# PRBonn/RAP

Measured on AMD Instinct MI355X. Metric: registered points/sec @20 flow steps, 2-view N=4096, higher is better.
Workload: dtype f32; 1 GPU; configs[1]: batch=32 samples/GPU x 2 views x 4096 pts, 20 Euler flow steps, rap_12 (d=512, H=8), fp32 (exact-fp32 MFMA), rigidity_forcing=on, final per-view SE(3) fit; preset=1, pairs_per_gpu=32, views=2, points_per_view=4096, flow_steps=20, num_layers=12, rigidity_forcing=True

## Files before the change

rap_amd/csrc/api.hip:

```cpp
#include "../../include/rapflow.h"
#include "half.h"
#include "kernels.h"

#include <mutex>
#include <new>
#include <vector>

static thread_local int g_last_hip_error = 0;
void rap_set_last_hip_error(int e) { g_last_hip_error = e; }

#define RAP_PROF_CLASSES 8
struct ProfRec { hipEvent_t a, b; int cls; };
static std::atomic<bool> g_prof_on{false};
static std::mutex g_prof_mu;
static std::vector<ProfRec> g_prof_recs;
static std::vector<hipEvent_t> g_prof_pool;
static size_t g_prof_pool_used = 0;
static const size_t RAP_PROF_MAX_EVENTS = 1u << 19;

static hipEvent_t prof_event() {
  if (g_prof_pool_used < g_prof_pool.size()) return g_prof_pool[g_prof_pool_used++];
  if (g_prof_pool.size() >= RAP_PROF_MAX_EVENTS) return nullptr;
  hipEvent_t e = nullptr;
  if (hipEventCreate(&e) != hipSuccess) return nullptr;
  g_prof_pool.push_back(e);
  g_prof_pool_used++;
  return e;
}
struct ProfScope {
  hipStream_t s; hipEvent_t a = nullptr, b = nullptr; int cls;
  ProfScope(hipStream_t s_, int cls_) : s(s_), cls(cls_) {
    if (!g_prof_on.load(std::memory_order_relaxed)) return;
    std::lock_guard<std::mutex> lock(g_prof_mu);
    a = prof_event(); b = prof_event();
    if (a && b) (void)hipEventRecord(a, s); else a = b = nullptr;
  }
  ~ProfScope() {
    if (a && b) {
      std::lock_guard<std::mutex> lock(g_prof_mu);
      (void)hipEventRecord(b, s); g_prof_recs.push_back({a, b, cls});
    }
  }
};
extern "C" int rap_profile_enable(int on) { g_prof_on.store(on != 0); return RAP_OK; }
extern "C" int rap_profile_reset(void) { std::lock_guard<std::mutex> lock(g_prof_mu); g_prof_recs.clear(); g_prof_pool_used = 0; return RAP_OK; }
extern "C" int rap_profile_collect_ex(float* h_ms_out, int64_t* h_count_out, int32_t n_classes) {
  if (!h_ms_out || !h_count_out || n_classes <= 0) return RAP_ERR_INVALID;
  std::lock_guard<std::mutex> lock(g_prof_mu);
  for (int c = 0; c < n_classes; ++c) { h_ms_out[c] = 0.f; h_count_out[c] = 0; }
  for (const ProfRec& r : g_prof_recs) {
    if (r.cls >= n_classes) continue;
    if (hipEventSynchronize(r.b) != hipSuccess) return RAP_ERR_HIP;
    float ms = 0.f;
    if (hipEventElapsedTime(&ms, r.a, r.b) != hipSuccess) return RAP_ERR_HIP;
    h_ms_out[r.cls] += ms; h_count_out[r.cls] += 1;
  }
  return RAP_OK;
}
extern "C" int rap_profile_collect(float* h_ms_out, int64_t* h_count_out) { return rap_profile_collect_ex(h_ms_out, h_count_out, 3); }

struct LayerW {
  const float* Wqkv[2];
  const float* Wout[2];
  const float* bout[2];
  const float* gq[2];
  const float* gk[2];
  const float* ffn_g;
  const float* ffn_b;
  const float* Wff1p;
  const float* bff1p;
  const float* Wff2;
  const float* bff2;
};

struct LayerWH {
  const u16* Wqkv[2];
  const u16* Wout[2];
  const u16* Wff1p;
  const u16* Wff2;
  float s_qkv[2] = {1.f, 1.f}, s_out[2] = {1.f, 1.f}, s_ff1 = 1.f, s_ff2 = 1.f;
  float g_v[2] = {1.f, 1.f}, g_ff1 = 1.f;
};
struct HalfWeights {
  u16* blob = nullptr;
  std::vector<LayerWH> layers;
};
#define RAP_MAX_LOGIT_BOUND 40.0f

struct rap_model {
  rap_model_desc desc;
  int d, L, H, F, E;
  int Din = 0;
  int Ks = 128;
  int dtype = RAP_DT_F32;
  bool qk_norm = true;
  int resid_dtype = RAP_DT_F32;
  HalfWeights half[4];
  float* logit_bound = nullptr;
  std::vector<uint8_t> bounded;
  int n_bounded = 0;
  float* raw = nullptr;
  float* derived = nullptr;
  const float* anchor_emb;
  const float* emb_bias;
  const float* Wstatic;
  const float* Wx;
  const float *adaW1, *adab1, *adaW2, *adab2, *adaW3, *adab3;
  std::vector<LayerW> layers;
  const float *hW0, *hb0, *hW2, *hb2, *hW4;
  mutable std::mutex cfg_mu;
};

static bool desc_ok(const rap_model_desc* d) {
  if (!d) return false;
  if (d->embed_dim <= 0 || d->embed_dim % 256 != 0 || d->embed_dim > 1024) return false;
  if (d->num_heads * 64 != d->embed_dim) return false;
  if (d->num_layers <= 0 || d->num_layers > 64) return false;
  if (d->local_feat_dim < 0 || d->local_feat_dim % 4 != 0 || d->local_feat_dim > 40) return false;
  return true;
}

extern rap_tuning_t g_rap_gemm_variant;
extern rap_tuning_t g_rap_gemm_stagger;
extern rap_tuning_t g_rap_gemm_splitk;
extern rap_tuning_t g_rap_geglu_fast;
extern rap_tuning_t g_rap_attn_split;
extern rap_tuning_t g_rap_gemm_h16_variant;
extern rap_tuning_t g_rap_attn_h16_variant;
extern rap_tuning_t g_rap_gemm_h16_persistent;
extern rap_tuning_t g_rap_attn_h16_dma;
extern rap_tuning_t g_rap_gemm_f32_persistent;
extern rap_tuning_t g_rap_attn_x2_wpe;
extern rap_tuning_t g_rap_attn_h16_small;
rap_tuning_t g_rap_attn_lpt = 1;
rap_tuning_t g_rap_x2_min_rows = 1024;
rap_tuning_t g_rap_small_fused = 1;
extern rap_tuning_t g_rap_ring_blocks;
rap_tuning_t g_rap_fuse_qknorm = 1;
struct TuningRow { int32_t key; rap_tuning_t* var; int n_values; int32_t values[7]; };
static const TuningRow kTuning[] = {
#ifdef RAP_ABLATION_BUILD
  {0, &g_rap_gemm_variant, 3, {16, 32, 48}},
  {2, &g_rap_gemm_h16_variant, 3, {0, 1, 14}},
  {3, &g_rap_attn_h16_variant, 2, {0, 5}},
  {4, &g_rap_gemm_stagger, 3, {0, 1, 2}},
#endif
  {5, &g_rap_attn_split, 2, {0, 1}},
  {6, &g_rap_gemm_splitk, 2, {0, 1}},
  {7, &g_rap_fuse_qknorm, 2, {0, 1}},
  {9, &g_rap_geglu_fast, 2, {0, 1}},
  {11, &g_rap_gemm_h16_persistent, 2, {0, 1}},
  {12, &g_rap_gemm_f32_persistent, 2, {0, 1}},
  {13, &g_rap_attn_h16_dma, 2, {0, 1}},
  {15, &g_rap_attn_lpt, 2, {0, 1}},
  {16, &g_rap_attn_x2_wpe, 2, {2, 4}},
  {17, &g_rap_x2_min_rows, -1, {}},
  {18, &g_rap_ring_blocks, -1, {}},
  {19, &g_rap_small_fused, 2, {0, 1}},
  {20, &g_rap_attn_h16_small, 7, {0, 1, 2, 64, 128, 66, 130}},
};
extern "C" int rap_set_tuning(int32_t key, int32_t value) {
  for (const TuningRow& r : kTuning) {
    if (r.key != key) continue;
    bool ok = r.n_values < 0 && value >= 0;
    for (int i = 0; i < r.n_values; ++i) ok = ok || r.values[i] == value;
    if (ok) *r.var = value;
    return ok ? RAP_OK : RAP_ERR_INVALID;
  }
  return RAP_ERR_INVALID;
}

extern "C" int rap_version(void) { return RAPFLOW_ABI_VERSION; }
extern "C" int rap_last_hip_error(void) { return g_last_hip_error; }

static bool in_dim_ok(int32_t in_dim) { return in_dim >= 0 && in_dim <= 512 && in_dim % 4 == 0; }
extern "C" int64_t rap_weight_count(const rap_model_desc* desc) { return rap_weight_count_latent(desc, 0); }
extern "C" int64_t rap_weight_count_latent(const rap_model_desc* desc, int32_t in_dim) {
  if (!desc_ok(desc) || !in_dim_ok(in_dim)) return -1;
  const int64_t d = desc->embed_dim, L = desc->num_layers, H = desc->num_heads, E = 147 + desc->local_feat_dim + in_dim;
  int64_t n = 2 * d + d * E + d;
  const int64_t attn = (d * 256 + d) + (d * d + d) + (2 * d * d + 2 * d) + 3 * d * d + (d * d + d) + 2 * H * 64;
  const int64_t layer = 2 * attn + 2 * d + (8 * d * d + 8 * d) + (4 * d * d + d);
  n += L * layer;
  n += (d * d + d) + (d / 2 * d + d / 2) + 3 * (d / 2);
  return n;
}

static int ensure_logit_bounds(rap_model* m, hipStream_t stream);

extern "C" int rap_model_create(const rap_model_desc* desc, const float* d_weights, int64_t n_floats, void* stream_,
                                rap_model** out) {
  return rap_model_create_latent(desc, 0, d_weights, n_floats, stream_, out);
}
extern "C" int rap_model_create_latent(const rap_model_desc* desc, int32_t in_dim, const float* d_weights, int64_t n_floats, void* stream_,
                                       rap_model** out) {
  if (!out) return RAP_ERR_INVALID;
  *out = nullptr;
  if (!desc_ok(desc) || !in_dim_ok(in_dim) || !d_weights) return RAP_ERR_INVALID;
  if (n_floats != rap_weight_count_latent(desc, in_dim)) return RAP_ERR_INVALID;
  hipStream_t stream = (hipStream_t)stream_;
  rap_model* m = new (std::nothrow) rap_model();
  if (!m) return RAP_ERR_ALLOC;
  m->desc = *desc;
  const int d = m->d = desc->embed_dim, L = m->L = desc->num_layers, H = m->H = desc->num_heads;
  m->F = desc->local_feat_dim;
  m->Din = in_dim;
  const int Ks = m->Ks = 128 + (in_dim + 31) / 32 * 32;
  const int E = m->E = 147 + m->F + m->Din;
  if (hipMalloc((void**)&m->raw, (size_t)n_floats * sizeof(float)) != hipSuccess) { delete m; return RAP_ERR_ALLOC; }
  const size_t n_ada = (size_t)2 * L * ((size_t)d * 256 + d + (size_t)d * d + d + (size_t)2 * d * d + 2 * d);
  const size_t n_ff1 = (size_t)L * ((size_t)8 * d * d + 8 * d);
  const size_t n_derived = (size_t)d * Ks + (size_t)d * 64 + n_ada + n_ff1;
  if (hipMalloc((void**)&m->derived, n_derived * sizeof(float)) != hipSuccess) {
    (void)hipFree(m->raw); delete m; return RAP_ERR_ALLOC;
  }
  int rc = RAP_OK;
  auto fail = [&](int code) { rap_model_destroy(m); return code; };
  if (hipMemcpyAsync(m->raw, d_weights, (size_t)n_floats * sizeof(float), hipMemcpyDeviceToDevice, stream) != hipSuccess)
    return fail(RAP_ERR_HIP);

  const float* p = m->raw;
  auto take = [&](size_t n) { const float* r = p; p += n; return r; };
  m->anchor_emb = take((size_t)2 * d);
  const float* embW = take((size_t)d * E);
  m->emb_bias = take(d);

  float* q = m->derived;
  auto carve = [&](size_t n) { float* r = q; q += n; return r; };
  float* Wstatic = carve((size_t)d * Ks);
  float* Wx = carve((size_t)d * 64);
  float* aW1 = carve((size_t)2 * L * d * 256); float* ab1 = carve((size_t)2 * L * d);
  float* aW2 = carve((size_t)2 * L * d * d);   float* ab2 = carve((size_t)2 * L * d);
  float* aW3 = carve((size_t)2 * L * 2 * d * d); float* ab3 = carve((size_t)2 * L * 2 * d);
  m->Wstatic = Wstatic; m->Wx = Wx;
  m->adaW1 = aW1; m->adab1 = ab1; m->adaW2 = aW2; m->adab2 = ab2; m->adaW3 = aW3; m->adab3 = ab3;

  if ((rc = launch_fill_zero(stream, Wstatic, (size_t)d * Ks))) return fail(rc);
  if ((rc = launch_fill_zero(stream, Wx, (size_t)d * 64))) return fail(rc);
  if ((rc = launch_copy_cols(stream, embW, E, 0, Wstatic, Ks, 0, d, 63))) return fail(rc);
  if ((rc = launch_copy_cols(stream, embW, E, 126, Wstatic, Ks, 63, d, 21))) return fail(rc);
  if ((rc = launch_copy_cols(stream, embW, E, 147, Wstatic, Ks, 84, d, m->F))) return fail(rc);
  if ((rc = launch_copy_cols(stream, embW, E, 147 + m->F, Wstatic, Ks, 128, d, m->Din))) return fail(rc);
  if ((rc = launch_copy_cols(stream, embW, E, 63, Wx, 64, 0, d, 63))) return fail(rc);

  m->layers.resize(L);
  for (int i = 0; i < L; ++i) {
    LayerW& lw = m->layers[i];
    for (int a = 0; a < 2; ++a) {
      const int j = 2 * i + a;
      const float* W1 = take((size_t)d * 256); const float* b1 = take(d);
      const float* W2 = take((size_t)d * d);   const float* b2 = take(d);
      const float* W3 = take((size_t)2 * d * d); const float* b3 = take((size_t)2 * d);
      if ((rc = launch_copy_cols(stream, W1, 256, 0, aW1 + (size_t)j * d * 256, 256, 0, d, 256))) return fail(rc);
      if ((rc = launch_copy_cols(stream, b1, d, 0, ab1 + (size_t)j * d, d, 0, 1, d))) return fail(rc);
      if ((rc = launch_copy_cols(stream, W2, d, 0, aW2 + (size_t)j * d * d, d, 0, d, d))) return fail(rc);
      if ((rc = launch_copy_cols(stream, b2, d, 0, ab2 + (size_t)j * d, d, 0, 1, d))) return fail(rc);
      if ((rc = launch_copy_cols(stream, W3, d, 0, aW3 + (size_t)j * 2 * d * d, d, 0, 2 * d, d))) return fail(rc);
      if ((rc = launch_copy_cols(stream, b3, 2 * d, 0, ab3 + (size_t)j * 2 * d, 2 * d, 0, 1, 2 * d))) return fail(rc);
      lw.Wqkv[a] = take((size_t)3 * d * d);
      lw.Wout[a] = take((size_t)d * d);
      lw.bout[a] = take(d);
      lw.gq[a] = take((size_t)H * 64);
      lw.gk[a] = take((size_t)H * 64);
    }
    lw.ffn_g = take(d);
    lw.ffn_b = take(d);
    const float* Wff1 = take((size_t)8 * d * d);
    const float* bff1 = take((size_t)8 * d);
    float* Wp = carve((size_t)8 * d * d);
    float* bp = carve((size_t)8 * d);
    if ((rc = launch_geglu_interleave(stream, Wff1, bff1, Wp, bp, 4 * d, d))) return fail(rc);
    lw.Wff1p = Wp; lw.bff1p = bp;
    lw.Wff2 = take((size_t)d * 4 * d);
    lw.bff2 = take(d);
  }
  m->hW0 = take((size_t)d * d); m->hb0 = take(d);
  m->hW2 = take((size_t)(d / 2) * d); m->hb2 = take(d / 2);
  m->hW4 = take((size_t)3 * (d / 2));
  if ((int64_t)(p - m->raw) != n_floats || (size_t)(q - m->derived) != n_derived) return fail(RAP_ERR_INVALID);
  if ((rc = ensure_logit_bounds(m, stream))) return fail(rc);
  *out = m;
  return RAP_OK;
}

extern "C" void rap_model_destroy(rap_model* m) {
  if (!m) return;
  if (m->raw) (void)hipFree(m->raw);
  if (m->derived) (void)hipFree(m->derived);
  for (int i = 0; i < 4; ++i)
    if (m->half[i].blob) (void)hipFree(m->half[i].blob);
  if (m->logit_bound) (void)hipFree(m->logit_bound);
  delete m;
}

static int ensure_logit_bounds(rap_model* m, hipStream_t stream) {
  if (m->logit_bound) return RAP_OK;
  const int n = m->L * 2 * m->H;
  if (hipMalloc((void**)&m->logit_bound, (size_t)n * sizeof(float)) != hipSuccess) { m->logit_bound = nullptr; return RAP_ERR_ALLOC; }
  for (int i = 0; i < m->L; ++i)
    for (int a = 0; a < 2; ++a) {
      const int rc = launch_qk_logit_bound(stream, m->layers[i].gq[a], m->layers[i].gk[a], m->H, m->logit_bound + (size_t)(2 * i + a) * m->H);
      if (rc) return rc;
    }
  std::vector<float> hb(n);
  RAP_HIP_CHECK(hipMemcpyAsync(hb.data(), m->logit_bound, (size_t)n * sizeof(float), hipMemcpyDeviceToHost, stream));
  RAP_HIP_CHECK(hipStreamSynchronize(stream));
  m->bounded.assign((size_t)2 * m->L, 1);
  for (int j = 0; j < 2 * m->L; ++j)
    for (int h = 0; h < m->H; ++h)
      if (!(hb[(size_t)j * m->H + h] <= RAP_MAX_LOGIT_BOUND)) m->bounded[j] = 0;
  m->n_bounded = 0;
  for (uint8_t b : m->bounded) m->n_bounded += b;
  return RAP_OK;
}

static int build_x2_weights(rap_model* m, hipStream_t stream) {
  HalfWeights& hw = m->half[RAP_DT_F32X2];
  const size_t d = m->d, L = m->L;
  const size_t per_layer = 2 * (2 * (3 * d * d + d * d) + 8 * d * d + 4 * d * d);
  const int nt = (int)(6 * L);
  float* d_max = nullptr;
  if (hipMalloc((void**)&d_max, (size_t)nt * sizeof(float)) != hipSuccess) return RAP_ERR_ALLOC;
  if (hipMalloc((void**)&hw.blob, per_layer * L * sizeof(u16)) != hipSuccess) { hw.blob = nullptr; (void)hipFree(d_max); return RAP_ERR_ALLOC; }
  int rc = RAP_OK;
  auto fail = [&](int code) { (void)hipFree(hw.blob); hw.blob = nullptr; hw.layers.clear(); (void)hipFree(d_max); return code; };
  if (hipMemsetAsync(d_max, 0, (size_t)nt * sizeof(float), stream) != hipSuccess) return fail(RAP_ERR_HIP);
  struct Item { const float* src; size_t rows, cols; };
  std::vector<Item> items;
  for (size_t i = 0; i < L; ++i) {
    const LayerW& lw = m->layers[i];
    for (int a = 0; a < 2; ++a) { items.push_back({lw.Wqkv[a], 3 * d, d}); items.push_back({lw.Wout[a], d, d}); }
    items.push_back({lw.Wff1p, 8 * d, d});
    items.push_back({lw.Wff2, d, 4 * d});
  }
  for (int k = 0; k < nt && rc == RAP_OK; ++k) rc = launch_max_abs(stream, items[k].src, items[k].rows * items[k].cols, d_max + k);
  if (rc) return fail(rc);
  std::vector<float> hmax(nt);
  if (hipMemcpyAsync(hmax.data(), d_max, (size_t)nt * sizeof(float), hipMemcpyDeviceToHost, stream) != hipSuccess) return fail(RAP_ERR_HIP);
  if (hipStreamSynchronize(stream) != hipSuccess) return fail(RAP_ERR_HIP);
  u16* q = hw.blob;
  std::vector<const u16*> planes(nt);
  std::vector<float> inv(nt);
  std::vector<int> expo(nt);
  for (int k = 0; k < nt && rc == RAP_OK; ++k) {
    if (!(hmax[k] < 3.0e38f)) return fail(RAP_ERR_INVALID);
    int e = 0;
    if (hmax[k] > 0.f) { int ex; (void)frexpf(hmax[k], &ex); e = 12 - ex; }
    e = e > 60 ? 60 : e < -60 ? -60 : e;
    expo[k] = hmax[k] > 0.f ? e : 16;
    inv[k] = ldexpf(1.0f, -e);
    planes[k] = q;
    rc = launch_x2_pack(stream, items[k].src, (long)items[k].cols, (long)items[k].rows, (int)items[k].cols, ldexpf(1.0f, e), q);
    q += 2 * items[k].rows * items[k].cols;
  }
  if (rc) return fail(rc);
  hw.layers.resize(L);
  for (size_t i = 0; i < L; ++i) {
    LayerWH& lh = hw.layers[i];
    const int k0 = (int)(6 * i);
    for (int a = 0; a < 2; ++a) {
      lh.Wqkv[a] = planes[k0 + 2 * a]; lh.s_qkv[a] = inv[k0 + 2 * a];
      { int g = expo[k0 + 2 * a] - 16; g = g > 12 ? 12 : g < -12 ? -12 : g; lh.g_v[a] = ldexpf(1.0f, g); }
      lh.Wout[a] = planes[k0 + 2 * a + 1]; lh.s_out[a] = inv[k0 + 2 * a + 1];
    }
    lh.Wff1p = planes[k0 + 4]; lh.s_ff1 = inv[k0 + 4];
    { int g = 2 * (expo[k0 + 4] - 16); g = g > 24 ? 24 : g < -24 ? -24 : g; lh.g_ff1 = ldexpf(1.0f, g); }
    lh.Wff2 = planes[k0 + 5]; lh.s_ff2 = inv[k0 + 5];
  }
  (void)hipFree(d_max);
  return RAP_OK;
}

extern "C" int rap_model_set_compute_dtype(rap_model* m, int32_t dtype, void* stream_) {
  if (!m) return RAP_ERR_INVALID;
  std::lock_guard<std::mutex> lock(m->cfg_mu);
  if (dtype == RAP_DT_F32) { m->dtype = dtype; return RAP_OK; }
  if (dtype != RAP_DT_BF16 && dtype != RAP_DT_F16 && dtype != RAP_DT_F32X2) return RAP_ERR_INVALID;
  HalfWeights& hw = m->half[dtype];
  if (!hw.blob && dtype == RAP_DT_F32X2) {
    const int rcx = build_x2_weights(m, (hipStream_t)stream_);
    if (rcx) return rcx;
  }
  if (!hw.blob) {
    hipStream_t stream = (hipStream_t)stream_;
    const size_t d = m->d, L = m->L;
    const size_t per_layer = 2 * (3 * d * d + d * d) + 8 * d * d + 4 * d * d;
    if (hipMalloc((void**)&hw.blob, per_layer * L * sizeof(u16)) != hipSuccess) { hw.blob = nullptr; return RAP_ERR_ALLOC; }
    u16* q = hw.blob;
    int rc = RAP_OK;
    auto conv = [&](const float* src, size_t n) -> const u16* {
      u16* dst = q; q += n;
      if (rc == RAP_OK) rc = launch_convert_h16(stream, dtype, src, dst, n);
      return dst;
    };
    hw.layers.resize(L);
    for (size_t i = 0; i < L; ++i) {
      const LayerW& lw = m->layers[i];
      LayerWH& lh = hw.layers[i];
      for (int a = 0; a < 2; ++a) {
        lh.Wqkv[a] = conv(lw.Wqkv[a], 3 * d * d);
        lh.Wout[a] = conv(lw.Wout[a], d * d);
      }
      lh.Wff1p = conv(lw.Wff1p, 8 * d * d);
      lh.Wff2 = conv(lw.Wff2, 4 * d * d);
    }
    if (rc != RAP_OK) { (void)hipFree(hw.blob); hw.blob = nullptr; hw.layers.clear(); return rc; }
  }
  { const int rcb = ensure_logit_bounds(m, (hipStream_t)stream_); if (rcb) return rcb; }
  m->dtype = dtype;
  return RAP_OK;
}
extern "C" int rap_model_compute_dtype(const rap_model* m) { return m ? m->dtype : RAP_ERR_INVALID; }
extern "C" int rap_model_set_residual_dtype(rap_model* m, int32_t dtype) {
  if (!m || (dtype != RAP_DT_F32 && dtype != RAP_DT_F16)) return RAP_ERR_INVALID;
  std::lock_guard<std::mutex> lock(m->cfg_mu);
  m->resid_dtype = dtype;
  return RAP_OK;
}
extern "C" int rap_model_residual_dtype(const rap_model* m) { return m ? m->resid_dtype : RAP_ERR_INVALID; }
extern "C" int rap_model_bounded_attention_launches(const rap_model* m) { return m ? (m->qk_norm ? m->n_bounded : 0) : RAP_ERR_INVALID; }
extern "C" int rap_model_set_qk_norm(rap_model* m, int32_t on) {
  if (!m) return RAP_ERR_INVALID;
  std::lock_guard<std::mutex> lock(m->cfg_mu);
  m->qk_norm = on != 0;
  return RAP_OK;
}
extern "C" int rap_model_qk_norm(const rap_model* m) { return m ? (m->qk_norm ? 1 : 0) : RAP_ERR_INVALID; }

static int eff_dtype(const rap_model* m, size_t rows) {
  return (m->dtype == RAP_DT_F32X2 && (long)rows < (long)g_rap_x2_min_rows) ? RAP_DT_F32 : m->dtype;
}

struct Workspace {
  float *base, *h, *xn, *qkv, *att, *ffmid, *ax, *v, *mod, *ada_scratch, *xt, *Rc, *tc, *tgrid;
  u16* h16;
  float *hid1, *hid2, *astatic;
  u16 *xnh, *qkh, *vth, *atth, *ffmidh;
  float* splitk_h;
  int splitk_planes;
  int vt_nblk;
  int rows;
  int dtype;
  bool qk_norm;
  double* proc_partials;
  int32_t *token_sample, *part_offsets, *attn_sort;
  int32_t *cu_batch_s, *cu_part_s;
  const int32_t* cu_part_live;
  int nseg_part, nseg_batch;
  AttnWorkItem *items_batch, *items_part;
  int max_items_batch, max_items_part;
  int attn_bq;
  int attn_kg;
  size_t total;
};

static Workspace carve_workspace(const rap_model* m, int64_t TP, int B, int nseg_part, int rows, char* basep, int force_dtype = -1) {
  Workspace w;
  const size_t d = m->d, L = m->L;
  Carver c(basep);
  const size_t T = align_up((size_t)TP, 256);
  w.rows = (int)T;
  const int dtype = w.dtype = force_dtype >= 0 ? force_dtype : eff_dtype(m, T);
// ... 450 lines not shown
```

rap_amd/csrc/attn_f32.hip:

```cpp
#include "kernels.h"

#define AQ_WAVE 64
#define AKV 64
#define KLD 68
#define VLD 64
#define ATTN_FENCE __builtin_amdgcn_sched_barrier(0x406);

__device__ __forceinline__ float xhalf_max(float v) {
  const auto r = __builtin_amdgcn_permlane32_swap(__float_as_uint(v), __float_as_uint(v), false, false);
  return fmaxf(__uint_as_float(r[0]), __uint_as_float(r[1]));
}
__device__ __forceinline__ float xhalf_sum(float v) {
  const auto r = __builtin_amdgcn_permlane32_swap(__float_as_uint(v), __float_as_uint(v), false, false);
  return __uint_as_float(r[0]) + __uint_as_float(r[1]);
}

#define ATTN_DEFER_THR 11.5f
__device__ __forceinline__ float amax3(float a, float b, float c) {
  float r;
  asm("v_max3_f32 %0, %1, %2, %3" : "=v"(r) : "v"(a), "v"(b), "v"(c));
  return r;
}

template <int NW, bool BOUNDED, bool SPLIT = false>
__global__ __launch_bounds__(64 * NW, 2) void attention_f32_kernel(const float* __restrict__ qkv, float* __restrict__ out,
                                                                  int TP, int heads, const AttnWorkItem* __restrict__ items,
                                                                  const float* __restrict__ bound, float* __restrict__ part_o,
                                                                  float* __restrict__ part_l) {
  __shared__ __attribute__((aligned(16))) float smem[2 * AKV * KLD + 2 * AKV * VLD];
  float* Ks = smem;
  float* Vs = smem + 2 * AKV * KLD;

  const int head = blockIdx.x % heads;
  const AttnWorkItem it = items[blockIdx.x / heads];
  const int len = it.seg_len;
  if (len <= 0) return;
  const int tid = threadIdx.x;
  const int lane = tid & 63, wave = tid >> 6;
  const int hi = lane >> 5, l31 = lane & 31;

  const size_t plane = (size_t)heads * TP * 64;
  const float* Qg = qkv + ((size_t)head * TP + it.seg_start) * 64;
  const float* Kg = Qg + plane;
  const float* Vg = Qg + 2 * plane;

  const int qw0 = it.q0 + wave * AQ_WAVE;
  const bool wave_active = qw0 < len;
  if (NW == 8) {
    if (__builtin_amdgcn_readfirstlane(threadIdx.x) >= 256) __builtin_amdgcn_s_setprio(1);
  }

  const float qscale = 0.125f * 1.44269504088896340736f;
  float qf[2][32];
#pragma unroll
  for (int qt = 0; qt < 2; ++qt) {
    int q = qw0 + qt * 32 + l31;
    q = q < len ? q : len - 1;
    const float* qp = Qg + (size_t)q * 64 + 4 * hi;
#pragma unroll
    for (int g = 0; g < 8; ++g) {
      const float4 v = *reinterpret_cast<const float4*>(qp + 8 * g);
      qf[qt][g * 4 + 0] = v.x * qscale;
      qf[qt][g * 4 + 1] = v.y * qscale;
      qf[qt][g * 4 + 2] = v.z * qscale;
      qf[qt][g * 4 + 3] = v.w * qscale;
    }
  }

  f32x16 o[2][2];
#pragma unroll
  for (int a = 0; a < 2; ++a)
#pragma unroll
    for (int b = 0; b < 2; ++b)
#pragma unroll
      for (int r = 0; r < 16; ++r) o[a][b][r] = 0.f;
  const bool bound_ok = BOUNDED ? (bound[head] <= 40.0f) : true;
  float mrun[2] = {-1e30f, -1e30f};
  float lsum[2] = {0.f, 0.f};

  constexpr int RS = 4 * NW;
  const int srow = tid >> 4;
  const int sc4 = (tid & 15) * 4;
  float4 rk0, rk1, rk2, rk3, rv0, rv1, rv2, rv3;
  const int nkv = (len + AKV - 1) / AKV;
  int t_begin = 0, t_end = nkv;
  if (SPLIT) {
    t_begin = (int)((long)nkv * blockIdx.y / gridDim.y);
    t_end = (int)((long)nkv * (blockIdx.y + 1) / gridDim.y);
  }
  const int koff = srow * KLD + sc4;
  const int voff = srow * VLD + sc4;

#define ATTN_LOAD_ONE(T, I, RK, RV)                                          \
  {                                                                          \
    int key_ = (T) * AKV + srow + RS * (I);                                  \
    key_ = key_ < len ? key_ : len - 1;                                      \
    RK = *reinterpret_cast<const float4*>(Kg + (size_t)key_ * 64 + sc4);     \
    RV = *reinterpret_cast<const float4*>(Vg + (size_t)key_ * 64 + sc4);     \
  }
#define ATTN_LOAD_TILE(T)          \
  ATTN_LOAD_ONE(T, 0, rk0, rv0)    \
  ATTN_LOAD_ONE(T, 1, rk1, rv1)    \
  if constexpr (NW == 4) {         \
    ATTN_LOAD_ONE(T, 2, rk2, rv2)  \
    ATTN_LOAD_ONE(T, 3, rk3, rv3)  \
  }
#define ATTN_STORE_ONE(BUF, I, RK, RV)                                                            \
  *reinterpret_cast<float4*>(&Ks[(BUF) * (AKV * KLD) + koff + RS * (I) * KLD]) = RK;              \
  *reinterpret_cast<float4*>(&Vs[(BUF) * (AKV * VLD) + voff + RS * (I) * VLD]) = RV;
#define ATTN_STORE_TILE(BUF)           \
  ATTN_STORE_ONE(BUF, 0, rk0, rv0)     \
  ATTN_STORE_ONE(BUF, 1, rk1, rv1)     \
  if constexpr (NW == 4) {             \
    ATTN_STORE_ONE(BUF, 2, rk2, rv2)   \
    ATTN_STORE_ONE(BUF, 3, rk3, rv3)   \
  }

  ATTN_LOAD_TILE(t_begin)
  ATTN_STORE_TILE(0)
  __syncthreads();

  for (int t = t_begin; t < t_end; ++t) {
    const int cur = (t - t_begin) & 1;
    const bool more = (t + 1) < t_end;
    if (more) { ATTN_LOAD_TILE(t + 1) }

    if (wave_active) {
      const float* Kc = Ks + cur * (AKV * KLD);
      const float* Vc = Vs + cur * (AKV * VLD);
#pragma unroll
      for (int kt = 0; kt < 2; ++kt) {
        const int kbase = t * AKV + kt * 32;
        if (kbase >= len) break;
        f32x16 st[2];
#pragma unroll
        for (int r = 0; r < 16; ++r) { st[0][r] = 0.f; st[1][r] = 0.f; }
        const float* kp = Kc + (kt * 32 + l31) * KLD + 4 * hi;
        const float* vp = Vc + (kt * 32 + 4 * hi) * VLD + 2 * l31;
        float4 kf = *reinterpret_cast<const float4*>(kp);
        float2 vfa, vfb;
#pragma unroll
        for (int g = 0; g < 8; ++g) {
          float4 kn = kf;
          if (g < 7) kn = *reinterpret_cast<const float4*>(kp + 8 * (g + 1));
          else { vfa = *reinterpret_cast<const float2*>(vp); vfb = *reinterpret_cast<const float2*>(vp + VLD); }
          ATTN_FENCE
          st[0] = __builtin_amdgcn_mfma_f32_32x32x2f32(kf.x, qf[0][g * 4 + 0], st[0], 0, 0, 0);
          st[1] = __builtin_amdgcn_mfma_f32_32x32x2f32(kf.x, qf[1][g * 4 + 0], st[1], 0, 0, 0);
          st[0] = __builtin_amdgcn_mfma_f32_32x32x2f32(kf.y, qf[0][g * 4 + 1], st[0], 0, 0, 0);
          st[1] = __builtin_amdgcn_mfma_f32_32x32x2f32(kf.y, qf[1][g * 4 + 1], st[1], 0, 0, 0);
          st[0] = __builtin_amdgcn_mfma_f32_32x32x2f32(kf.z, qf[0][g * 4 + 2], st[0], 0, 0, 0);
          st[1] = __builtin_amdgcn_mfma_f32_32x32x2f32(kf.z, qf[1][g * 4 + 2], st[1], 0, 0, 0);
          st[0] = __builtin_amdgcn_mfma_f32_32x32x2f32(kf.w, qf[0][g * 4 + 3], st[0], 0, 0, 0);
          st[1] = __builtin_amdgcn_mfma_f32_32x32x2f32(kf.w, qf[1][g * 4 + 3], st[1], 0, 0, 0);
          ATTN_FENCE
          kf = kn;
        }
        if (kbase + 32 > len) {
#pragma unroll
          for (int r = 0; r < 16; ++r) {
            const bool valid = (kbase + mfma32_crow(r, hi)) < len;
            st[0][r] = valid ? st[0][r] : -1e30f;
            st[1][r] = valid ? st[1][r] : -1e30f;
          }
        }
        if (BOUNDED) {
#pragma unroll
          for (int qt = 0; qt < 2; ++qt) {
            float pa = 0.f, pb2 = 0.f;
#pragma unroll
            for (int r = 0; r < 16; r += 2) {
              const float e0 = __builtin_amdgcn_exp2f(st[qt][r]);
              const float e1 = __builtin_amdgcn_exp2f(st[qt][r + 1]);
              st[qt][r] = e0; st[qt][r + 1] = e1;
              pa += e0; pb2 += e1;
            }
            lsum[qt] += pa + pb2;
          }
        } else {
#pragma unroll
        for (int qt = 0; qt < 2; ++qt) {
          float mx = amax3(st[qt][0], st[qt][1], st[qt][2]);
#pragma unroll
          for (int r = 3; r < 15; r += 2) mx = amax3(mx, st[qt][r], st[qt][r + 1]);
          mx = xhalf_max(fmaxf(mx, st[qt][15]));
          if (__builtin_amdgcn_ballot_w64(mx > mrun[qt] + ATTN_DEFER_THR) != 0) {
            const float mnew = fmaxf(mrun[qt], mx);
            const float alpha = __builtin_amdgcn_exp2f(mrun[qt] - mnew);
            mrun[qt] = mnew;
            lsum[qt] *= alpha;
#pragma unroll
            for (int r = 0; r < 16; ++r) {
              o[qt][0][r] *= alpha;
              o[qt][1][r] *= alpha;
            }
          }
          float pa = 0.f, pb2 = 0.f;
#pragma unroll
          for (int r = 0; r < 16; r += 2) {
            const float e0 = __builtin_amdgcn_exp2f(st[qt][r] - mrun[qt]);
            const float e1 = __builtin_amdgcn_exp2f(st[qt][r + 1] - mrun[qt]);
            st[qt][r] = e0; st[qt][r + 1] = e1;
            pa += e0; pb2 += e1;
          }
          lsum[qt] += pa + pb2;
        }
        }
#pragma unroll
        for (int r = 0; r < 16; r += 2) {
          float2 vna = vfa, vnb = vfb;
          if (r + 2 < 16) {
            const int k0 = ((r + 2) & 3) + 8 * ((r + 2) >> 2);
            const int k1 = ((r + 3) & 3) + 8 * ((r + 3) >> 2);
            vna = *reinterpret_cast<const float2*>(vp + k0 * VLD);
            vnb = *reinterpret_cast<const float2*>(vp + k1 * VLD);
          }
          ATTN_FENCE
          o[0][0] = __builtin_amdgcn_mfma_f32_32x32x2f32(vfa.x, st[0][r], o[0][0], 0, 0, 0);
          o[0][1] = __builtin_amdgcn_mfma_f32_32x32x2f32(vfa.y, st[0][r], o[0][1], 0, 0, 0);
          o[1][0] = __builtin_amdgcn_mfma_f32_32x32x2f32(vfa.x, st[1][r], o[1][0], 0, 0, 0);
          o[1][1] = __builtin_amdgcn_mfma_f32_32x32x2f32(vfa.y, st[1][r], o[1][1], 0, 0, 0);
          o[0][0] = __builtin_amdgcn_mfma_f32_32x32x2f32(vfb.x, st[0][r + 1], o[0][0], 0, 0, 0);
          o[0][1] = __builtin_amdgcn_mfma_f32_32x32x2f32(vfb.y, st[0][r + 1], o[0][1], 0, 0, 0);
          o[1][0] = __builtin_amdgcn_mfma_f32_32x32x2f32(vfb.x, st[1][r + 1], o[1][0], 0, 0, 0);
          o[1][1] = __builtin_amdgcn_mfma_f32_32x32x2f32(vfb.y, st[1][r + 1], o[1][1], 0, 0, 0);
          ATTN_FENCE
          vfa = vna; vfb = vnb;
        }
      }
    }

    if (more) { ATTN_STORE_TILE(cur ^ 1) }
    __syncthreads();
  }

  if (!wave_active) return;
  const int dmodel = heads * 64;
#pragma unroll
  for (int qt = 0; qt < 2; ++qt) {
    const int q = qw0 + qt * 32 + l31;
    const float ltot = xhalf_sum(lsum[qt]);
    const float inv = SPLIT ? 1.0f : (bound_ok ? 1.0f / ltot : __builtin_nanf(""));
    if (q < len) {
      float* op = (SPLIT ? part_o + (size_t)blockIdx.y * TP * dmodel : out) + (size_t)(it.seg_start + q) * dmodel + head * 64;
      if (SPLIT && hi == 0)
        part_l[((size_t)blockIdx.y * TP + it.seg_start + q) * heads + head] = bound_ok ? ltot : __builtin_nanf("");
#pragma unroll
      for (int rg = 0; rg < 4; ++rg) {
        const int d0 = 2 * (8 * rg + 4 * hi);
        float4 w0, w1;
        w0.x = o[qt][0][4 * rg + 0] * inv; w0.y = o[qt][1][4 * rg + 0] * inv;
        w0.z = o[qt][0][4 * rg + 1] * inv; w0.w = o[qt][1][4 * rg + 1] * inv;
        w1.x = o[qt][0][4 * rg + 2] * inv; w1.y = o[qt][1][4 * rg + 2] * inv;
        w1.z = o[qt][0][4 * rg + 3] * inv; w1.w = o[qt][1][4 * rg + 3] * inv;
        *reinterpret_cast<float4*>(op + d0) = w0;
        *reinterpret_cast<float4*>(op + d0 + 4) = w1;
      }
    }
  }
}

#define WL_THREADS 1024
#define WL_TILE 4096
#define WL_SORT_MAX 8192
__device__ __forceinline__ int wl_len(const int32_t* __restrict__ cu, int s) { const int l = cu[s + 1] - cu[s]; return l > 0 ? l : 0; }
__global__ __launch_bounds__(WL_THREADS) void build_attn_worklist_kernel(const int32_t* __restrict__ cu, int nseg, AttnWorkItem* __restrict__ items,
                                                                          int max_items, int bq, int32_t* __restrict__ sort_ws) {
  if (blockIdx.x != 0) return;
  const int tid = threadIdx.x;
  const AttnWorkItem none = {0, 0, 0, 0};
  if (!sort_ws) {
    if (tid != 0) return;
    int n = 0;
    for (int s = 0; s < nseg; ++s) {
      const int a = cu[s], len = wl_len(cu, s);
      for (int q0 = 0; q0 < len && n < max_items; q0 += bq) { const AttnWorkItem w = {a, len, q0, 0}; items[n++] = w; }
    }
    for (; n < max_items; ++n) items[n] = none;
    return;
  }
  __shared__ int lens[WL_TILE];
  __shared__ int partial[WL_THREADS];
  __shared__ int total_items;
  int32_t* order = sort_ws;
  if (nseg > WL_SORT_MAX) {
    for (int s = tid; s < nseg; s += WL_THREADS) order[s] = s;
  } else
  for (int s0 = 0; s0 < nseg; s0 += WL_THREADS) {
    const int s = s0 + tid;
    const int my = s < nseg ? wl_len(cu, s) : -1;
    int rank = 0;
    for (int j0 = 0; j0 < nseg; j0 += WL_TILE) {
      __syncthreads();
      for (int j = tid; j < WL_TILE && j0 + j < nseg; j += WL_THREADS) lens[j] = wl_len(cu, j0 + j);
      __syncthreads();
      const int nj = nseg - j0 < WL_TILE ? nseg - j0 : WL_TILE;
      if (s < nseg)
        for (int j = 0; j < nj; ++j) rank += (lens[j] > my || (lens[j] == my && j0 + j < s)) ? 1 : 0;
    }
    if (s < nseg) order[rank] = s;
  }
  __threadfence_block();
  __syncthreads();
  const int per = (nseg + WL_THREADS - 1) / WL_THREADS;
  const int r0 = tid * per, r1 = (r0 + per) < nseg ? (r0 + per) : nseg;
  int sum = 0;
  for (int r = r0; r < r1; ++r) { const int sg = order[r]; sum += (wl_len(cu, sg) + bq - 1) / bq; }
  partial[tid] = sum;
  __syncthreads();
  if (tid == 0) {
    int acc = 0;
    for (int t = 0; t < WL_THREADS; ++t) { const int v = partial[t]; partial[t] = acc; acc += v; }
    total_items = acc;
  }
  __syncthreads();
  int n = partial[tid];
  for (int r = r0; r < r1; ++r) {
    const int sg = order[r];
    const int a = cu[sg], len = wl_len(cu, sg);
    for (int q0 = 0; q0 < len; q0 += bq, ++n)
      if (n < max_items) { const AttnWorkItem w = {a, len, q0, 0}; items[n] = w; }
  }
  __syncthreads();
  const int total = total_items < 0 ? 0 : total_items < max_items ? total_items : max_items;
  for (int i = total + tid; i < max_items; i += WL_THREADS) items[i] = none;
}

rap_tuning_t g_rap_attn_variant = 1;
rap_tuning_t g_rap_attn_split = 1;
static int attn_block_queries() { return RAP_ATTN_BQ; }

int launch_build_attn_worklist(hipStream_t stream, const int32_t* cu_seqlens, int nseg, AttnWorkItem* items,
                               int max_items, int block_queries, int32_t* sort_ws) {
  if (max_items <= 0) return RAP_OK;
  hipLaunchKernelGGL(build_attn_worklist_kernel, dim3(1), dim3(WL_THREADS), 0, stream, cu_seqlens, nseg, items, max_items,
                     block_queries > 0 ? block_queries : attn_block_queries(), sort_ws);
  RAP_LAUNCH_CHECK();
  return RAP_OK;
}

__global__ __launch_bounds__(256) void attention_combine_kernel(const float* __restrict__ part_o, const float* __restrict__ part_l,
                                                                float* __restrict__ out, int TP, int heads, int splits,
                                                                const int32_t* __restrict__ cover_cu, int cover_nseg) {
  const int dmodel = heads * 64;
  const long i = (long)blockIdx.x * 256 + threadIdx.x;
  if (i >= (long)TP * dmodel / 4) return;
  const long t = i / (dmodel / 4);
  const int c = (int)(i % (dmodel / 4)) * 4;
  if (cover_cu && (t < cover_cu[0] || t >= cover_cu[cover_nseg])) {
    *reinterpret_cast<float4*>(out + t * dmodel + c) = float4{0.f, 0.f, 0.f, 0.f};
    return;
  }
  float4 acc = {0.f, 0.f, 0.f, 0.f};
  float l = 0.f;
  for (int s = 0; s < splits; ++s) {
    const float4 v = *reinterpret_cast<const float4*>(part_o + ((size_t)s * TP + t) * dmodel + c);
    acc.x += v.x; acc.y += v.y; acc.z += v.z; acc.w += v.w;
    l += part_l[((size_t)s * TP + t) * heads + (c >> 6)];
  }
  const float inv = l > 0.f ? 1.0f / l : 0.f;
  acc.x *= inv; acc.y *= inv; acc.z *= inv; acc.w *= inv;
  *reinterpret_cast<float4*>(out + t * dmodel + c) = acc;
}

int attention_f32_splits(int max_items, int heads, bool bounded) {
  if (!bounded || g_rap_attn_split == 0) return 1;
  const long blocks = (long)max_items * heads;
  return blocks <= 160 ? 4 : blocks <= 320 ? 2 : 1;
}

int launch_attention_f32(hipStream_t stream, const float* qkv, float* out, int TP, int heads, const AttnWorkItem* items,
                         int max_items, const float* bound, float* part_o, float* part_l, int splits, const int32_t* cover_cu,
                         int cover_nseg) {
  if (max_items <= 0 || TP <= 0) return RAP_OK;
  if (heads <= 0) return RAP_ERR_INVALID;
  if (splits > 1) {
    if (!bound || !part_o || !part_l) return RAP_ERR_INVALID;
    unsigned dyn = 0;
    if ((long)max_items * heads * splits <= 384) {
      dyn = 16384;
      if (hipFuncSetAttribute(reinterpret_cast<const void*>(attention_f32_kernel<4, true, true>), hipFuncAttributeMaxDynamicSharedMemorySize, dyn) != hipSuccess) {
        rap_set_last_hip_error((int)hipGetLastError());
        return RAP_ERR_HIP;
      }
    }
    hipLaunchKernelGGL((attention_f32_kernel<4, true, true>), dim3(max_items * heads, splits), dim3(256), dyn, stream, qkv, out, TP,
                       heads, items, bound, part_o, part_l);
    RAP_LAUNCH_CHECK();
    const long n4 = (long)TP * heads * 16;
    hipLaunchKernelGGL(attention_combine_kernel, dim3((unsigned)((n4 + 255) / 256)), dim3(256), 0, stream, part_o, part_l, out, TP,
                       heads, splits, cover_cu, cover_nseg);
    RAP_LAUNCH_CHECK();
    return RAP_OK;
  }
  float* const no = nullptr;
  if (bound) hipLaunchKernelGGL((attention_f32_kernel<4, true>), dim3(max_items * heads), dim3(256), 0, stream, qkv, out, TP, heads, items, bound, no, no);
  else hipLaunchKernelGGL((attention_f32_kernel<4, false>), dim3(max_items * heads), dim3(256), 0, stream, qkv, out, TP, heads, items, bound, no, no);
  RAP_LAUNCH_CHECK();
  return RAP_OK;
}
```

Baseline: 16300 points/s.

## Interleave next K/V tile prefetch and LDS stores into attention MFMA loop

```diff
diff --git a/rap_amd/csrc/api.hip b/rap_amd/csrc/api.hip
--- a/rap_amd/csrc/api.hip
+++ b/rap_amd/csrc/api.hip
@@ -125,6 +125,7 @@
 extern rap_tuning_t g_rap_gemm_splitk;
 extern rap_tuning_t g_rap_geglu_fast;
 extern rap_tuning_t g_rap_attn_split;
+extern rap_tuning_t g_rap_attn_sched;
 extern rap_tuning_t g_rap_gemm_h16_variant;
 extern rap_tuning_t g_rap_attn_h16_variant;
 extern rap_tuning_t g_rap_gemm_h16_persistent;
@@ -158,6 +159,7 @@
   {18, &g_rap_ring_blocks, -1, {}},
   {19, &g_rap_small_fused, 2, {0, 1}},
   {20, &g_rap_attn_h16_small, 7, {0, 1, 2, 64, 128, 66, 130}},
+  {21, &g_rap_attn_sched, 2, {0, 2}},
 };
 extern "C" int rap_set_tuning(int32_t key, int32_t value) {
   for (const TuningRow& r : kTuning) {
diff --git a/rap_amd/csrc/attn_f32.hip b/rap_amd/csrc/attn_f32.hip
--- a/rap_amd/csrc/attn_f32.hip
+++ b/rap_amd/csrc/attn_f32.hip
@@ -22,11 +22,23 @@
   return r;
 }
 
-template <int NW, bool BOUNDED, bool SPLIT = false>
-__global__ __launch_bounds__(64 * NW, 2) void attention_f32_kernel(const float* __restrict__ qkv, float* __restrict__ out,
-                                                                  int TP, int heads, const AttnWorkItem* __restrict__ items,
-                                                                  const float* __restrict__ bound, float* __restrict__ part_o,
-                                                                  float* __restrict__ part_l) {
+#ifdef RAP_ABLATION_BUILD
+#define ATTN_TS_BLOCKS 1024
+#define ATTN_TS_TILES 64
+__device__ unsigned long long* g_attn_ts = nullptr;
+extern "C" int rap_debug_attn_ts(void* p) { return hipMemcpyToSymbol(HIP_SYMBOL(g_attn_ts), &p, sizeof(p)) == hipSuccess ? 0 : -3; }
+#define ATTN_TS(I) { ATTN_FENCE ts[I] = __builtin_amdgcn_s_memtime(); ATTN_FENCE }
+#else
+#define ATTN_TS(I)
+#endif
+
+template <int NW, bool BOUNDED, bool SPLIT, int SCHED>
+__device__ __forceinline__ void attention_f32_block(const float* __restrict__ qkv, float* __restrict__ out,
+                                                    int TP, int heads, const AttnWorkItem* __restrict__ items,
+                                                    const float* __restrict__ bound, float* __restrict__ part_o,
+                                                    float* __restrict__ part_l) {
+  constexpr bool S_TILE = SCHED == 2;
+  static_assert(SCHED == 0 || (SCHED == 2 && NW == 4), "schedule 2 of tuning key 21 is written for the 4-wave block");
   __shared__ __attribute__((aligned(16))) float smem[2 * AKV * KLD + 2 * AKV * VLD];
   float* Ks = smem;
   float* Vs = smem + 2 * AKV * KLD;
@@ -105,6 +117,22 @@
     ATTN_LOAD_ONE(T, 2, rk2, rv2)  \
     ATTN_LOAD_ONE(T, 3, rk3, rv3)  \
   }
+  const unsigned last_off = (unsigned)(len - 1) * 256u + (unsigned)sc4 * 4u;
+  unsigned run_off = (unsigned)((t_begin + 1) * AKV + srow) * 256u + (unsigned)sc4 * 4u;
+#define ATTN_LOAD_ONE_RUN(I, RK, RV)                                                                   \
+  {                                                                                                    \
+    unsigned off_ = run_off + (unsigned)(RS * (I)) * 256u;                                             \
+    off_ = off_ < last_off ? off_ : last_off;                                                          \
+    RK = *reinterpret_cast<const float4*>(reinterpret_cast<const char*>(Kg) + off_);                   \
+    RV = *reinterpret_cast<const float4*>(reinterpret_cast<const char*>(Vg) + off_);                   \
+  }
+#define ATTN_LOAD_TILE_RUN           \
+  ATTN_LOAD_ONE_RUN(0, rk0, rv0)     \
+  ATTN_LOAD_ONE_RUN(1, rk1, rv1)     \
+  if constexpr (NW == 4) {           \
+    ATTN_LOAD_ONE_RUN(2, rk2, rv2)   \
+    ATTN_LOAD_ONE_RUN(3, rk3, rv3)   \
+  }
 #define ATTN_STORE_ONE(BUF, I, RK, RV)                                                            \
   *reinterpret_cast<float4*>(&Ks[(BUF) * (AKV * KLD) + koff + RS * (I) * KLD]) = RK;              \
   *reinterpret_cast<float4*>(&Vs[(BUF) * (AKV * VLD) + voff + RS * (I) * VLD]) = RV;
@@ -116,14 +144,36 @@
     ATTN_STORE_ONE(BUF, 3, rk3, rv3)   \
   }
 
+#define ATTN_STAGE_STEP(I, RK, RV)                                     \
+  if constexpr (S_TILE && NW == 4) {                                   \
+    if (g == 0) {                                                      \
+      ATTN_FENCE                                                       \
+      if (kt == 0) { ATTN_LOAD_ONE_RUN(I, RK, RV) }                    \
+      else { if ((I) == 0) { ATTN_TS(6) } ATTN_STORE_ONE(cur ^ 1, I, RK, RV) }   \
+      ATTN_FENCE                                                       \
+    }                                                                  \
+  }
+
   ATTN_LOAD_TILE(t_begin)
   ATTN_STORE_TILE(0)
   __syncthreads();
 
+#ifdef RAP_ABLATION_BUILD
+  unsigned long long ts[8] = {0, 0, 0, 0, 0, 0, 0, 0};
+  unsigned long long* ts_base = g_attn_ts;
+  if (blockIdx.x >= ATTN_TS_BLOCKS || (SPLIT && blockIdx.y != 0)) ts_base = nullptr;
+  if (ts_base && lane == 0)
+    ts_base[(size_t)ATTN_TS_BLOCKS * 4 * ATTN_TS_TILES * 8 + blockIdx.x * 4 + wave] =
+        ((unsigned long long)(__builtin_amdgcn_s_getreg((31 << 11) | 20) & 15u) << 16) | (__builtin_amdgcn_s_getreg((31 << 11) | 4) & 0xffffu);
+#endif
+
   for (int t = t_begin; t < t_end; ++t) {
     const int cur = (t - t_begin) & 1;
     const bool more = (t + 1) < t_end;
-    if (more) { ATTN_LOAD_TILE(t + 1) }
+    ATTN_TS(0)
+    if constexpr (!S_TILE) {
+      if (more) { ATTN_LOAD_TILE(t + 1) }
+    }
 
     if (wave_active) {
       const float* Kc = Ks + cur * (AKV * KLD);
@@ -147,15 +197,21 @@
           ATTN_FENCE
           st[0] = __builtin_amdgcn_mfma_f32_32x32x2f32(kf.x, qf[0][g * 4 + 0], st[0], 0, 0, 0);
           st[1] = __builtin_amdgcn_mfma_f32_32x32x2f32(kf.x, qf[1][g * 4 + 0], st[1], 0, 0, 0);
+          ATTN_STAGE_STEP(0, rk0, rv0)
           st[0] = __builtin_amdgcn_mfma_f32_32x32x2f32(kf.y, qf[0][g * 4 + 1], st[0], 0, 0, 0);
           st[1] = __builtin_amdgcn_mfma_f32_32x32x2f32(kf.y, qf[1][g * 4 + 1], st[1], 0, 0, 0);
+          ATTN_STAGE_STEP(1, rk1, rv1)
           st[0] = __builtin_amdgcn_mfma_f32_32x32x2f32(kf.z, qf[0][g * 4 + 2], st[0], 0, 0, 0);
           st[1] = __builtin_amdgcn_mfma_f32_32x32x2f32(kf.z, qf[1][g * 4 + 2], st[1], 0, 0, 0);
+          ATTN_STAGE_STEP(2, rk2, rv2)
           st[0] = __builtin_amdgcn_mfma_f32_32x32x2f32(kf.w, qf[0][g * 4 + 3], st[0], 0, 0, 0);
           st[1] = __builtin_amdgcn_mfma_f32_32x32x2f32(kf.w, qf[1][g * 4 + 3], st[1], 0, 0, 0);
+          ATTN_STAGE_STEP(3, rk3, rv3)
+          if (g == 0 && kt == 0) { ATTN_TS(1) }
           ATTN_FENCE
           kf = kn;
         }
+        ATTN_TS(2 + 2 * kt)
         if (kbase + 32 > len) {
 #pragma unroll
           for (int r = 0; r < 16; ++r) {
@@ -224,14 +280,31 @@
           o[0][1] = __builtin_amdgcn_mfma_f32_32x32x2f32(vfb.y, st[0][r + 1], o[0][1], 0, 0, 0);
           o[1][0] = __builtin_amdgcn_mfma_f32_32x32x2f32(vfb.x, st[1][r + 1], o[1][0], 0, 0, 0);
           o[1][1] = __builtin_amdgcn_mfma_f32_32x32x2f32(vfb.y, st[1][r + 1], o[1][1], 0, 0, 0);
+          if (r == 0) { ATTN_TS(3 + 2 * kt) }
           ATTN_FENCE
           vfa = vna; vfb = vnb;
         }
       }
-    }
-
-    if (more) { ATTN_STORE_TILE(cur ^ 1) }
+    } else if constexpr (S_TILE) {
+      ATTN_LOAD_TILE_RUN
+      if (more) { ATTN_STORE_TILE(cur ^ 1) }
+    }
+
+    if constexpr (!S_TILE) {
+      ATTN_TS(6)
+      if (more) { ATTN_STORE_TILE(cur ^ 1) }
+    } else {
+      run_off += AKV * 256u;
+    }
     __syncthreads();
+#ifdef RAP_ABLATION_BUILD
+    ATTN_TS(7)
+    if (ts_base && lane == 0 && t - t_begin < ATTN_TS_TILES) {
+      unsigned long long* dst = ts_base + (((size_t)blockIdx.x * 4 + wave) * ATTN_TS_TILES + (t - t_begin)) * 8;
+#pragma unroll
+      for (int i = 0; i < 8; ++i) dst[i] = ts[i];
+    }
+#endif
   }
 
   if (!wave_active) return;
@@ -258,6 +331,21 @@
       }
     }
   }
+}
+
+template <int NW, bool BOUNDED, bool SPLIT = false>
+__global__ __launch_bounds__(64 * NW, 2) void attention_f32_kernel(const float* __restrict__ qkv, float* __restrict__ out,
+                                                                  int TP, int heads, const AttnWorkItem* __restrict__ items,
+                                                                  const float* __restrict__ bound, float* __restrict__ part_o,
+                                                                  float* __restrict__ part_l) {
+  attention_f32_block<NW, BOUNDED, SPLIT, 2>(qkv, out, TP, heads, items, bound, part_o, part_l);
+}
+template <int NW, bool BOUNDED, bool SPLIT = false>
+__global__ __launch_bounds__(64 * NW, 2) void attention_f32_sched0_kernel(const float* __restrict__ qkv, float* __restrict__ out,
+                                                                         int TP, int heads, const AttnWorkItem* __restrict__ items,
+                                                                         const float* __restrict__ bound, float* __restrict__ part_o,
+                                                                         float* __restrict__ part_l) {
+  attention_f32_block<NW, BOUNDED, SPLIT, 0>(qkv, out, TP, heads, items, bound, part_o, part_l);
 }
 
 #define WL_THREADS 1024
@@ -328,6 +416,7 @@
 
 rap_tuning_t g_rap_attn_variant = 1;
 rap_tuning_t g_rap_attn_split = 1;
+rap_tuning_t g_rap_attn_sched = 2;
 static int attn_block_queries() { return RAP_ATTN_BQ; }
 
 int launch_build_attn_worklist(hipStream_t stream, const int32_t* cu_seqlens, int nseg, AttnWorkItem* items,
@@ -369,23 +458,30 @@
   return blocks <= 160 ? 4 : blocks <= 320 ? 2 : 1;
 }
 
+typedef void (*attn_f32_fn)(const float*, float*, int, int, const AttnWorkItem*, const float*, float*, float*);
+template <bool BOUNDED, bool SPLIT>
+static attn_f32_fn attn_f32_kernel_for(int sched) {
+  return sched != 0 ? attention_f32_kernel<4, BOUNDED, SPLIT> : attention_f32_sched0_kernel<4, BOUNDED, SPLIT>;
+}
+
 int launch_attention_f32(hipStream_t stream, const float* qkv, float* out, int TP, int heads, const AttnWorkItem* items,
                          int max_items, const float* bound, float* part_o, float* part_l, int splits, const int32_t* cover_cu,
                          int cover_nseg) {
   if (max_items <= 0 || TP <= 0) return RAP_OK;
   if (heads <= 0) return RAP_ERR_INVALID;
+  const int sched = TP <= (1 << 24) - 256 ? (int)g_rap_attn_sched.load() : 0;
   if (splits > 1) {
     if (!bound || !part_o || !part_l) return RAP_ERR_INVALID;
+    const attn_f32_fn fn = attn_f32_kernel_for<true, true>(sched);
     unsigned dyn = 0;
     if ((long)max_items * heads * splits <= 384) {
       dyn = 16384;
-      if (hipFuncSetAttribute(reinterpret_cast<const void*>(attention_f32_kernel<4, true, true>), hipFuncAttributeMaxDynamicSharedMemorySize, dyn) != hipSuccess) {
+      if (hipFuncSetAttribute(reinterpret_cast<const void*>(fn), hipFuncAttributeMaxDynamicSharedMemorySize, dyn) != hipSuccess) {
         rap_set_last_hip_error((int)hipGetLastError());
         return RAP_ERR_HIP;
       }
     }
-    hipLaunchKernelGGL((attention_f32_kernel<4, true, true>), dim3(max_items * heads, splits), dim3(256), dyn, stream, qkv, out, TP,
-                       heads, items, bound, part_o, part_l);
+    hipLaunchKernelGGL(fn, dim3(max_items * heads, splits), dim3(256), dyn, stream, qkv, out, TP, heads, items, bound, part_o, part_l);
     RAP_LAUNCH_CHECK();
     const long n4 = (long)TP * heads * 16;
     hipLaunchKernelGGL(attention_combine_kernel, dim3((unsigned)((n4 + 255) / 256)), dim3(256), 0, stream, part_o, part_l, out, TP,
@@ -394,8 +490,8 @@
     return RAP_OK;
   }
   float* const no = nullptr;
-  if (bound) hipLaunchKernelGGL((attention_f32_kernel<4, true>), dim3(max_items * heads), dim3(256), 0, stream, qkv, out, TP, heads, items, bound, no, no);
-  else hipLaunchKernelGGL((attention_f32_kernel<4, false>), dim3(max_items * heads), dim3(256), 0, stream, qkv, out, TP, heads, items, bound, no, no);
+  const attn_f32_fn fn = bound ? attn_f32_kernel_for<true, false>(sched) : attn_f32_kernel_for<false, false>(sched);
+  hipLaunchKernelGGL(fn, dim3(max_items * heads), dim3(256), 0, stream, qkv, out, TP, heads, items, bound, no, no);
   RAP_LAUNCH_CHECK();
   return RAP_OK;
 }
```

After: 16430 points/s (median of 6 runs). No clear change (+0.8%).
